# LongruiDong/nice-slam

Measured on AMD Instinct MI355X. Metric: ray-samples/sec (fwd+bwd) per mapping iter; frames/sec on Replica room0, higher is better.
Workload: dtype f32 (z, depth, var in f64); 1 GPU; Replica room0 mapping iteration, colour stage: 1000 pixels x 48 samples (5-frame window x 200), grids middle/fine/colour, Adam; global_batch=48000, seq_len=48, parallelism=rays sharded dp1, RCCL all-reduce of the frustum-row gradients

## Files before the change

include/nslam.h:

```cpp
#ifndef NSLAM_H
#define NSLAM_H

#include <stddef.h>
#include <stdint.h>

#ifdef __cplusplus
extern "C" {
#endif

#define NSLAM_C_DIM 32
#define NSLAM_HIDDEN 32
#define NSLAM_EMB 93

enum {
  NSLAM_OK = 0,
  NSLAM_EINVAL = -1,
  NSLAM_EUNSUPPORTED = -2,
  NSLAM_EWORKSPACE = -3,
  NSLAM_EHIP = -1000
};

enum { NSLAM_STAGE_COARSE = 0, NSLAM_STAGE_MIDDLE = 1, NSLAM_STAGE_FINE = 2, NSLAM_STAGE_COLOR = 3 };
enum { NSLAM_DEC_COARSE = 0, NSLAM_DEC_MIDDLE = 1, NSLAM_DEC_FINE = 2, NSLAM_DEC_COLOR = 3 };
enum { NSLAM_FWD_DEFAULT = 0, NSLAM_FWD_UNITS = 1, NSLAM_FWD_PC = 2, NSLAM_FWD_PARTS = 3 };
// ... 47 lines not shown
int nslam_query_fwd_ws(const nslam_query_cfg* cfg, const double* pts, int64_t n_pts, float* raw, void* ws,
                       size_t ws_bytes, void* stream);
size_t nslam_query_fwd_workspace_size(const nslam_query_cfg* cfg, int64_t n_pts);

int nslam_query_bwd(const nslam_query_cfg* cfg, const double* pts, int64_t n_pts, const float* g_raw,
                    double* g_pts, void* ws, size_t ws_bytes, void* stream);
size_t nslam_query_bwd_workspace_size(const nslam_query_cfg* cfg, int64_t n_pts);
int nslam_query_bwd_decoder(const nslam_query_cfg* cfg, int32_t dec, int32_t accumulate_pts, const double* pts,
                            int64_t n_pts, const float* g_raw, double* g_pts, void* ws, size_t ws_bytes,
                            void* stream);
size_t nslam_query_bwd_decoder_workspace_size(const nslam_query_cfg* cfg, int32_t dec, int64_t n_pts);
size_t nslam_query_saved_size(int64_t n_pts);
size_t nslam_query_tape_size(int64_t n_pts);
int nslam_query_bwd_decoders(const nslam_query_cfg* cfg, int32_t dec_mask, const double* pts, int64_t n_pts,
                             const float* g_raw, double* const* g_pts, void* stream);
int nslam_color_wgrad(const nslam_query_cfg* cfg, const double* pts, int64_t n_pts, const float* g_raw, void* ws,
                      size_t ws_bytes, void* stream);

int nslam_composite_fwd(const float* raw, const double* z_vals, int64_t n_rays, int32_t n_samples,
                        double* depth, double* var, float* color, void* stream);
int nslam_composite_bwd(const float* raw, const double* z_vals, int64_t n_rays, int32_t n_samples,
                        const double* g_depth, const double* g_var, const float* g_color, float* g_raw,
                        void* stream);

int nslam_grid_sample_fwd(const float* grid, const int32_t* dims, const float* coords, int64_t n,
                          float* out, void* stream);
int nslam_grid_sample_bwd(const float* grid, const int32_t* dims, const float* coords, int64_t n,
                          const float* grad_out, float* grad_grid, float* grad_coords, void* stream);

#define NSLAM_MAX_FRAMES 32
// ... 140 lines not shown
```

nice-slam_amd/_lib.py:

```python
from __future__ import annotations

import ctypes
import os

import torch

_HERE = os.path.dirname(os.path.abspath(__file__))
LIB_PATH = os.environ.get("NSLAM_LIB") or os.path.join(_HERE, "libnslam.so")

NSLAM_OK = 0
ABI_VERSION = 23
STAGES = {"coarse": 0, "middle": 1, "fine": 2, "color": 3}
DEC_COARSE, DEC_MIDDLE, DEC_FINE, DEC_COLOR = 0, 1, 2, 3

c_float_p = ctypes.POINTER(ctypes.c_float)


class NslamGrid(ctypes.Structure):
    _fields_ = [
        ("data", ctypes.c_void_p),
        ("grad", ctypes.c_void_p),
        ("dims", ctypes.c_int32 * 3),
        ("pad_", ctypes.c_int32),
        ("lo", ctypes.c_double * 3),
# ... 87 lines not shown

EXPORTS = (
    "nslam_pack_layout", "nslam_sample_rays", "nslam_query_fwd", "nslam_query_bwd", "nslam_query_bwd_workspace_size",
    "nslam_query_saved_size", "nslam_query_bwd_decoder", "nslam_query_bwd_decoder_workspace_size",
    "nslam_query_bwd_decoders",
    "nslam_composite_fwd", "nslam_composite_bwd", "nslam_grid_sample_fwd", "nslam_grid_sample_bwd",
    "nslam_workspace_size", "nslam_strerror", "nslam_abi_version", "nslam_gather_rays", "nslam_render_loss",
    "nslam_render_loss_workspace_size", "nslam_adam_step", "nslam_rows_pack", "nslam_rows_unpack",
    "nslam_query_fwd_ws", "nslam_query_fwd_workspace_size", "nslam_cam_grad", "nslam_cam_pose",
    "nslam_query_tape_size", "nslam_color_wgrad", "nslam_cam_grad_parts", "nslam_cam_grad_batch",
    "nslam_cam_pose_batch", "nslam_frustum_rows", "nslam_frustum_rows_workspace_size", "nslam_track_best",
    "nslam_loss_sum_best", "nslam_cam_vector_batch", "nslam_cam_grad_step",
    "nslam_point_masks", "nslam_point_masks_workspace_size", "nslam_mc_count", "nslam_mc_emit",
    "nslam_mc_workspace_size", "nslam_points_in_hull", "nslam_mesh_face_cull", "nslam_mesh_components",
    "nslam_mesh_select", "nslam_mesh_remap",
)

_lib = None


def lib():
    global _lib
    if _lib is None:
        if not os.path.exists(LIB_PATH):
            raise RuntimeError(f"{LIB_PATH} is missing: build it with __graft_entry__.build() "
                               "(make -C nice-slam_amd/csrc); there is no CPU fallback")
        L = ctypes.CDLL(LIB_PATH)
        missing = [n for n in EXPORTS if not hasattr(L, n)]
        if missing:
            raise RuntimeError(f"{LIB_PATH} does not export {', '.join(missing)}: rebuild it "
# ... 53 lines not shown
                                          vp, vp, vp, vp]
        f64 = ctypes.c_double
        L.nslam_point_masks.argtypes = [vp, i64, vp, i32, vp, i32, i32, f32, f32, f32, f32, i32, i32, i64, vp, vp, vp,
                                        vp, sz, vp]
        L.nslam_point_masks_workspace_size.argtypes = [i64, i32, i64]
        L.nslam_point_masks_workspace_size.restype = sz
        L.nslam_mc_count.argtypes = [vp, i32, i32, i32, f32, vp, sz, vp]
        L.nslam_mc_emit.argtypes = [vp, i32, i32, i32, f32, dp, dp, vp, vp, i64, i64, vp, vp, vp]
        L.nslam_mc_workspace_size.argtypes = [i32, i32, i32]
        L.nslam_mc_workspace_size.restype = sz
        L.nslam_points_in_hull.argtypes = [vp, i32, i64, vp, i32, vp, vp]
        L.nslam_mesh_face_cull.argtypes = [vp, i64, vp, i64, vp, vp]
        L.nslam_mesh_components.argtypes = [vp, i64, vp, i64, vp, vp, vp, vp]
        L.nslam_mesh_select.argtypes = [vp, i64, vp, vp, vp, f64, vp, vp, vp]
        L.nslam_mesh_remap.argtypes = [vp, i64, vp, vp, vp]
        if L.nslam_abi_version() != ABI_VERSION:
            raise RuntimeError(f"libnslam.so ABI {L.nslam_abi_version()} != {ABI_VERSION}: rebuild it")
        _lib = L
    return _lib


def check(rc: int, what: str):
    if rc != NSLAM_OK:
        msg = lib().nslam_strerror(rc).decode()
        raise RuntimeError(f"{what} failed: rc={rc} ({msg})")


def ptr(t):
    if t is None:
        return None
# ... 16 lines not shown
```

nice-slam_amd/csrc/nslam_query_impl.h:

```cpp
#pragma once
#include <type_traits>

#include "nslam_dev.h"

namespace nslamq {

struct QueryKArgs {
  nslam_query_cfg c;
  const double* pts;
  int64_t n;
  float* raw;
  const float* g_raw;
  double* g_pts;
};

struct Pt {
  double p[3];
  float x[3];
  bool valid;
  bool inside;
};

__device__ __forceinline__ Pt load_point(const QueryKArgs& a, int64_t idx) {
  Pt q;
// ... 267 lines not shown
__device__ __forceinline__ uint16_t* mask_slot(const QueryKArgs& a, int dec, int64_t tile) {
  const int64_t ntiles = (a.n + 31) / 32;
  return a.c.saved_masks + ((size_t)dec * ntiles + tile) * 5 * 64;
}
__device__ __forceinline__ void save_masks(const QueryKArgs& a, int dec, int64_t tile, const uint32_t m[5],
                                           int lane) {
  if (!a.c.saved_masks) return;
  uint16_t* s = mask_slot(a, dec, tile);
#pragma unroll
  for (int i = 0; i < 5; ++i) s[i * 64 + lane] = (uint16_t)m[i];
}
__device__ __forceinline__ void load_masks(const QueryKArgs& a, int dec, int64_t tile, uint32_t m[5], int lane) {
  const uint16_t* s = mask_slot(a, dec, tile);
#pragma unroll
  for (int i = 0; i < 5; ++i) m[i] = s[i * 64 + lane];
}

constexpr int kTapeFloats = 5 * 16 * 64;
__device__ __forceinline__ void tape_store(float* __restrict__ t, int i, const f32x16& v, int lane) {
  const int p = lane & 31, h = lane >> 5;
  __attribute__((address_space(1))) f32x4* q =
      reinterpret_cast<__attribute__((address_space(1))) f32x4*>(as_global_w(t) + i * 1024 + p * 32 + 4 * h);
#pragma unroll
  for (int k = 0; k < 4; ++k) q[2 * k] = f32x4{v[4 * k], v[4 * k + 1], v[4 * k + 2], v[4 * k + 3]};
}
struct Slab {
  __amdgpu_buffer_rsrc_t r;
};

__device__ __forceinline__ Slab make_slab(float* base, int floats) {
// ... 1321 lines not shown
static __global__ __launch_bounds__(256) void k_occ_combine(float* __restrict__ raw, const float* __restrict__ occ_mid,
                                                     int64_t n) {
  const int64_t p = (int64_t)blockIdx.x * 256 + threadIdx.x;
  if (p < n) raw[p * 4 + 3] = raw[p * 4 + 3] + occ_mid[p];
}

constexpr int kScratchFloats = 2 * TILE_FLOATS + 32 * 4 + 32 * 3 + 32 * 8 * 2 + 32;
constexpr int kWavesBwd = 4;
constexpr int kMaxSlabs = 4096;

constexpr bool lean_tr(int WG, bool PG, bool SAVED) { return SAVED && WG == 0 && !PG; }
constexpr int bwd_scratch_floats(int WG, bool PG, bool SAVED) {
  return WG ? kScratchFloats : lean_tr(WG, PG, SAVED) ? kWalkFloats : TILE_FLOATS + kWalkFloats;
}

template <int DEC, int WG, bool PG, bool FIRST, bool SAVED>
__device__ __forceinline__ void dec_bwd_tile(const QueryKArgs& a, int64_t tile, const Slab& A, const Scratch& S,
                                             int lane, double* __restrict__ gpts, int64_t gbase = 0) {
  asm volatile("" : "+v"(lane));
  PHASE(DEC, 0);
  const int h = lane >> 5, p = lane & 31;
  const int64_t idx = tile * 32 + p;
  const Pt q = load_point(a, idx);
  float g[4] = {0.f, 0.f, 0.f, 0.f};
  if (q.valid) {
    const f32x4 v = *reinterpret_cast<const f32x4*>(a.g_raw + idx * 4);
    g[0] = v[0];
    g[1] = v[1];
    g[2] = v[2];
    g[3] = q.inside ? v[3] : 0.f;
  }
  if (WG) {
    if (h == 0) {
#pragma unroll
      for (int j = 0; j < 4; ++j) S.gtab[p * 4 + j] = g[j];
#pragma unroll
      for (int j = 0; j < 3; ++j) S.xtab[p * 3 + j] = q.x[j];
// ... 8 lines not shown
  PHASE(DEC, 1);
  Corners cr;
  grid_corners(cr, gr, q);
  ScatterCorners scn{};
  if (WG == 0 && gr.grad) scn = resolve_corners(gr.slot, cr, q.valid, lane);
  PHASE(DEC, 2);
  f32x16 dc;
  float gx[3] = {0.f, 0.f, 0.f};
  static_assert(!(SAVED && WG), "weight gradients from saved masks run as k_color_wgrad");
  constexpr bool TR = lean_tr(WG, PG, SAVED);
  float* const tab = TR ? S.sA : S.sA + TILE_FLOATS;
  constexpr bool IMGDC = SAVED && WG == 0 && PG && DEC != NSLAM_DEC_COARSE;
  float* const img = IMGDC ? S.sA : nullptr;
  if (SAVED) {
    uint32_t m[5];
    load_masks(a, DEC, tile, m, lane);
    if (WG == 0 && gr.grad) stage_walk_table(tab, scn, cr.cell, lane);
    if (DEC == NSLAM_DEC_COARSE) {
      noxyz_backward_saved<TR>(pk, m, g[3], lane, dc);
    } else if (DEC == NSLAM_DEC_FINE) {
      xyz_backward_saved<2, 1, 3, PG, TR>(pk, m, q.x, g, lane, dc, gx, nullptr, img);
    } else if (DEC == NSLAM_DEC_COLOR) {
      xyz_backward_saved<1, 3, 0, PG, TR>(pk, m, q.x, g, lane, dc, gx, gh4, img);
    } else {
      xyz_backward_saved<1, 1, 3, PG, TR>(pk, m, q.x, g, lane, dc, gx, nullptr, img);
    }
  } else if (DEC == NSLAM_DEC_COARSE) {
    const f32x16 c = gather_tile(gr.data, cr, lane);
    noxyz_backward<WG>(pk, c, g[3], dg, A, S, lane, dc);
  } else if (DEC == NSLAM_DEC_FINE) {
    Corners cm;
// ... 80 lines not shown
      f32x4 t = s0[i];
      for (int v = 1; v < nv; ++v) t += s0[(size_t)v * q + i];
      s0[i] = t;
    }
    return;
  }
#pragma nounroll
  for (int64_t tile = w; tile < ntiles; tile += (int64_t)gridDim.x * kWavesBwd)
    dec_bwd_tile<DEC, WG, PG, FIRST, SAVED>(a, tile, A, S, lane, a.g_pts);
}

struct MultiDecArgs {
  int ndec;
  int dec[4];
  double* gp[4];
};
#ifndef NSLAM_MULTI_LB
#define NSLAM_MULTI_LB 4
#endif
#ifndef NSLAM_MULTI_PG_LB
#define NSLAM_MULTI_PG_LB 3
#endif
template <bool PG>
__global__ __launch_bounds__(64 * kWavesBwd, PG ? NSLAM_MULTI_PG_LB : NSLAM_MULTI_LB) void k_dec_bwd_multi(QueryKArgs a, MultiDecArgs m) {
  constexpr int kScr = bwd_scratch_floats(0, PG, true);
  __shared__ __attribute__((aligned(16))) float lds[kWavesBwd * kScr];
  const int lane = threadIdx.x & 63, wave = wave_id();
  Scratch S;
  S.sA = lds + wave * kScr;
  S.sX = S.gtab = S.xtab = S.cw = nullptr;
  S.crow = S.ccell = nullptr;
  const int part = (int)(blockIdx.x % (unsigned)m.ndec);
  const int dec = part == 0 ? m.dec[0] : part == 1 ? m.dec[1] : part == 2 ? m.dec[2] : m.dec[3];
  double* gp = part == 0 ? m.gp[0] : part == 1 ? m.gp[1] : part == 2 ? m.gp[2] : m.gp[3];
  const int64_t w = (int64_t)(blockIdx.x / (unsigned)m.ndec) * kWavesBwd + wave;
  const int64_t ntiles = (a.n + 31) / 32;
  if (w >= ntiles) return;
  TL(1, 0, part);
  const Slab A = make_slab(nullptr, 0);
  switch (dec) {
    case NSLAM_DEC_COARSE: dec_bwd_tile<NSLAM_DEC_COARSE, 0, PG, true, true>(a, w, A, S, lane, gp); break;
    case NSLAM_DEC_MIDDLE: dec_bwd_tile<NSLAM_DEC_MIDDLE, 0, PG, true, true>(a, w, A, S, lane, gp); break;
    case NSLAM_DEC_FINE: dec_bwd_tile<NSLAM_DEC_FINE, 0, PG, true, true>(a, w, A, S, lane, gp); break;
    default: dec_bwd_tile<NSLAM_DEC_COLOR, 0, PG, true, true>(a, w, A, S, lane, gp); break;
  }
  TL(1, 1, 0);
}

constexpr int kReduceWaves = 16;
static __global__ __launch_bounds__(64 * kReduceWaves) void k_slab_reduce(const float* __restrict__ slab, int64_t nslab,
                                                                   int acc_floats, int count,
                                                                   float* __restrict__ base) {
  __shared__ f32x4 part[kReduceWaves * 4][16];
  const int lane = threadIdx.x & 63, wave = wave_id();
  const int c = lane & 15, r = wave * 4 + (lane >> 4);
  const int j = (blockIdx.x * 16 + c) * 4;
  f32x4 s0 = {0.f, 0.f, 0.f, 0.f}, s1 = s0;
  if (j < count) {
    const float* p = slab + j;
// ... 188 lines not shown
```

nice-slam_amd/csrc/nslam_query_multi.hip:

```cpp
#include "nslam_query_impl.h"

using namespace nslamq;

extern "C" int nslam_query_bwd_decoders(const nslam_query_cfg* cfg, int32_t dec_mask, const double* pts,
                                        int64_t n_pts, const float* g_raw, double* const* g_pts, void* stream) {
  const int rc = check_cfg(cfg, true);
  if (rc) return rc;
  if (dec_mask <= 0 || dec_mask > 15) return NSLAM_EINVAL;
  if (n_pts < 0 || (n_pts > 0 && ((!pts && !cfg->rays_o) || !g_raw))) return NSLAM_EINVAL;
  if (cfg->rays_o && (n_pts >= (int64_t(1) << 31) || n_pts % cfg->n_samples)) return NSLAM_EINVAL;
  if (cfg->need_pts_grad && n_pts > 0 && !g_pts) return NSLAM_EINVAL;
  MultiDecArgs m{};
  for (int d = 0; d < 4; ++d) {
    if (!((dec_mask >> d) & 1)) continue;
    if (!stage_uses(cfg->stage, d)) return NSLAM_EINVAL;
    if (cfg->dgrad[d].base) return NSLAM_EUNSUPPORTED;
    if (cfg->need_pts_grad && n_pts > 0 && !g_pts[d]) return NSLAM_EINVAL;
    m.dec[m.ndec] = d;
    m.gp[m.ndec] = cfg->need_pts_grad ? g_pts[d] : nullptr;
    ++m.ndec;
  }
  if (n_pts > 0 && !cfg->saved_masks) return NSLAM_EUNSUPPORTED;
  if (n_pts == 0) return NSLAM_OK;
  const int64_t tiles = (n_pts + 31) / 32;
  const int64_t groups = (tiles + kWavesBwd - 1) / kWavesBwd;
  QueryKArgs a{*cfg, pts, n_pts, nullptr, g_raw, nullptr};
  hipStream_t s = reinterpret_cast<hipStream_t>(stream);
  const dim3 grid((unsigned)(groups * m.ndec)), block(64 * kWavesBwd);
  if (cfg->need_pts_grad)
    hipLaunchKernelGGL((k_dec_bwd_multi<true>), grid, block, 0, s, a, m);
  else
    hipLaunchKernelGGL((k_dec_bwd_multi<false>), grid, block, 0, s, a, m);
  return hip_status();
}

extern "C" int nslam_color_wgrad(const nslam_query_cfg* cfg, const double* pts, int64_t n_pts, const float* g_raw,
                                 void* ws, size_t ws_bytes, void* stream) {
  const int rc = check_cfg(cfg, true);
  if (rc) return rc;
  if (cfg->stage != NSLAM_STAGE_COLOR || n_pts < 0) return NSLAM_EINVAL;
  if (!cfg->dgrad[NSLAM_DEC_COLOR].base || cfg->dgrad[NSLAM_DEC_COLOR].count <= 0) return NSLAM_EUNSUPPORTED;
  if (n_pts > 0 && !cw_tape_path(cfg)) return NSLAM_EUNSUPPORTED;
  if (n_pts > 0 && ((!pts && !cfg->rays_o) || !g_raw)) return NSLAM_EINVAL;
  if (cfg->rays_o && (n_pts >= (int64_t(1) << 31) || n_pts % cfg->n_samples)) return NSLAM_EINVAL;
  if (n_pts == 0) return NSLAM_OK;
  if (!ws || ws_bytes < dec_ws_bytes(cfg, NSLAM_DEC_COLOR, n_pts)) return NSLAM_EWORKSPACE;
  QueryKArgs a{*cfg, pts, n_pts, nullptr, g_raw, nullptr};
  return launch_color_wgrad(a, reinterpret_cast<float*>(ws), reinterpret_cast<hipStream_t>(stream));
}
```

nice-slam_amd/engine.py:

```python
from __future__ import annotations

import ctypes
import math
import os
import weakref

import numpy as np
import torch

from . import _lib, ops
from ._lib import check, lib, ptr, stream_ptr
from .common import get_camera_from_tensor

_GRID_OF = {"coarse": "grid_coarse", "middle": "grid_middle", "fine": "grid_fine", "color": "grid_color"}


def _env_choice(name, default, allowed):
    v = os.environ.get(name, default)
    if v not in allowed:
        raise ValueError(f"{name}={v!r}: expected one of {sorted(allowed)}")
    return v


class FlatDecoder:
# ... 39 lines not shown
                 rows=None):
        self.nice, self.c, self.bound = nice, c, bound
        self.n_strat, self.n_surf, self.lindisp, self.w_color = n_strat, n_surf, lindisp, w_color
        self.device = torch.device(device)
        names = [n for n in ("coarse", "middle", "fine", "color") if hasattr(nice, n + "_decoder")]
        self.decs = {n: FlatDecoder(nice.decoder(n)) for n in names}
        self.dec_bounds = {n: ops._bound_list(nice.decoder(n).bound) for n in names}
        self.oob = ops._bound_list(bound)
        self._saved = None
        self._tape = None
        self.occ_add = None
        self._draws = None
        self._pre = None
        self._parity = 0
        self._pre_stream = None
        self._side = []
        self.concurrent = True
        self.wgrad_first = _env_choice("NSLAM_WGRAD_FIRST", "1", ("0", "1")) == "1"
        self.merge = True
        self._lean_ev = None
        self.prefetch_at = _env_choice("NSLAM_PREFETCH_AT", "start", ("start", "after_fwd"))
        self.prefetch_stream = _env_choice("NSLAM_PREFETCH_STREAM", "lean", ("lean", "own"))
        self.adam_merge = _env_choice("NSLAM_ADAM_MERGE", "1", ("0", "1")) == "1"
        self.adam_on = _env_choice("NSLAM_ADAM_ON", "side", ("side", "main"))
        self._wg_ev = None
        for k, v in c.items():
            if not v.is_contiguous(memory_format=torch.channels_last_3d):
                raise ValueError(f"{k} must be channels-last (ops.channels_last)")
        self.grid_grads = grid_grads
        self.layout_gen = 0
        self.pad_rows = 1
        self.set_rows(rows)

    def set_rows(self, rows, pad_rows=None):
        c = self.c
        pad = max(1, int(self.pad_rows if pad_rows is None else pad_rows))
        self.layout_gen += 1
        rup = lambda n: -(-n // pad) * pad
        drup = lambda n: -(-n // (32 * pad)) * 32 * pad
        self.rows = dict(rows) if rows else {}
# ... 36 lines not shown
        keys = tuple(sorted(masks))
        if getattr(self, "_cap_keys", None) != keys:
            self._cap = {}
            rows = {}
            for k in keys:
                n = self.c[k].numel() // 32
                full = torch.empty(n + 1, dtype=torch.int32, device=self.device)
                full[:n] = torch.arange(n, dtype=torch.int32, device=self.device)
                self._cap[k] = (full, torch.full((1,), n, dtype=torch.int64, device=self.device),
                                torch.arange(n, dtype=torch.int32, device=self.device))
                rows[k] = full[:n]
            self.set_rows(rows, pad_rows=1)
            self._cap_keys = keys
            self.gall.zero_()
            self._clean = True
        for k in keys:
            full, n_live, ar = self._cap[k]
            n = ar.numel()
            m = masks[k]
            if m is None:
                full[:n].copy_(ar)
                self.slot[k].copy_(ar)
                n_live.fill_(n)
                continue
            m = m.permute(2, 1, 0).reshape(-1)
            idx = torch.cumsum(m, 0, dtype=torch.int32) - 1
            self.slot[k].copy_(torch.where(m, idx, torch.full_like(idx, -1)))
            full.scatter_(0, torch.where(m, idx, torch.full_like(idx, n)).long(), ar)
            n_live.copy_(idx[-1:].to(torch.int64) + 1)
        return {k: self._cap[k][1] for k in keys}
# ... 7 lines not shown
        meta = ops.QueryMeta(stage, decs, {n: self.decs[n].packer for n in decs},
                             {n: self.dec_bounds[n] for n in decs}, self.oob, None)
        pairs = [(None, None, None)] * 4
        for n in decs:
            key = _GRID_OF[n]
            gg = key in grid_grads
            pairs[ops._DEC_ID[n]] = (self.c[key], self.ggrad[key] if gg else None, self.slot.get(key) if gg else None)
        packed = {n: self.decs[n].packed for n in decs}
        dg = {n: self.decs[n].grad for n in decs if n in dec_grads}
        cfg = ops._fill_cfg(meta, pairs, packed, dg, False)
        cfg.rays_o, cfg.rays_d, cfg.z_vals, cfg.n_samples = ptr(ro), ptr(rd), ptr(z), z.shape[1]
        cfg.saved_masks = ptr(self._saved)
        cfg.act_tape = ptr(self._tape)
        return cfg

    def query_fwd(self, stage, ro, rd, z, defer_occ=False, tape=False):
        n = z.numel()
        raw = torch.empty(n, 4, dtype=torch.float32, device=z.device)
        self._saved = torch.empty(lib().nslam_query_saved_size(n), dtype=torch.uint8, device=z.device)
        self._tape = None
        if tape and stage == "color":
            self._tape = torch.empty(lib().nslam_query_tape_size(n) // 4, dtype=torch.float32, device=z.device)
        cfg = self._cfg(stage, ro, rd, z, (), ())
        self.occ_add = ops.query_fwd_launch(cfg, None, n, raw, defer_occ=defer_occ)
        return raw

    def query_bwd(self, stage, ro, rd, z, g_raw, grid_grads, dec_grads, concurrent=None, pts_grad=False,
                  on_branch=None, pts_parts=False, ordered_branches=False, on_pts=None):
        n = z.numel()
        self._clean = False
        concurrent = self.concurrent if concurrent is None else concurrent
        cfg = self._cfg(stage, ro, rd, z, grid_grads, dec_grads)
        cfg.need_pts_grad = int(bool(pts_grad))
        decs = list(ops._DEC_FOR_STAGE[stage])
        wgt = [d for d in decs if d in dec_grads]
        masks = self._saved is not None
        tape_color = "color" in wgt and masks and self._tape is not None
        lean = [d for d in decs if self.merge and masks and (d not in wgt or (d == "color" and tape_color))]
        others = [d for d in decs if d not in lean]
        gp = {d: torch.empty(n, 3, dtype=torch.float64, device=z.device) for d in decs} if pts_grad else None
        units = []
        if "color" in lean and "color" in wgt and n > 0:
            units.append(("wgrad", ["color"]))
        if lean:
            units.append(("lean", lean))
        units += [("one", [d]) for d in others]
        if not self.wgrad_first:
            units.sort(key=lambda u: u[0] == "wgrad")
# ... 1 lines not shown
        merged_names = None
        merge_adam = (self.adam_merge and has_wgrad and on_branch is not None and not ordered_branches
                      and self.wgrad_first and concurrent and len(units) == 2 and units[1][0] == "lean")
        wgrad_st = None
        main = torch.cuda.current_stream(z.device)
        par = concurrent and len(units) > 1
        streams = [main]
        if par:
            while len(self._side) < len(units) - 1:
                self._side.append(torch.cuda.Stream(z.device))
            streams += self._side[:len(units) - 1]
        used = streams[1:]
        with ops._span("query_bwd"):
            for st in used:
                st.wait_stream(main)
                for t in (ro, rd, z, g_raw, self._saved, self._tape):
                    if t is not None:
                        t.record_stream(st)
            for i, (kind, names) in enumerate(units):
                st = streams[i] if par else main
                with torch.cuda.stream(st):
                    if kind == "wgrad":
                        wsb = lib().nslam_query_bwd_decoder_workspace_size(ctypes.byref(cfg), _lib.DEC_COLOR, n)
                        ws = torch.empty(wsb, dtype=torch.uint8, device=z.device)
                        with ops._span("query_bwd.color_wgrad"):
                            rc = lib().nslam_color_wgrad(ctypes.byref(cfg), None, n, ptr(g_raw), ptr(ws), wsb,
                                                         st.cuda_stream)
                        check(rc, "nslam_color_wgrad")
                        wgrad_st = st
                        if merge_adam:
                            if self._wg_ev is None:
                                self._wg_ev = torch.cuda.Event()
                            self._wg_ev.record(st)
                    elif kind == "lean":
                        lc = _lib.NslamQueryCfg.from_buffer_copy(cfg)
                        gps = (ctypes.c_void_p * 4)()
                        mask = 0
                        for name in names:
                            d = ops._DEC_ID[name]
                            mask |= 1 << d
                            lc.dgrad[d] = _lib.NslamDecGrad()
                            if pts_grad:
                                gps[d] = ptr(gp[name])
                        with ops._span("query_bwd." + "+".join(names)):
                            rc = lib().nslam_query_bwd_decoders(ctypes.byref(lc), mask, None, n, ptr(g_raw), gps,
                                                                st.cuda_stream)
                        check(rc, "nslam_query_bwd_decoders")
                        if on_pts is not None and pts_grad and set(names) == set(decs):
                            for name in names:
                                gp[name].record_stream(st)
                            on_pts([gp[d] for d in decs])
                            on_pts = None
                        if has_wgrad and self._lean_ev is None:
                            self._lean_ev = torch.cuda.Event()
                        if has_wgrad and not ordered_branches:
                            self._lean_ev.record(st)
                        if on_branch is not None and merge_adam and self.adam_on == "main":
                            merged_names = names
                        elif on_branch is not None and merge_adam:
                            st.wait_event(self._wg_ev)
                            on_branch(names, part="all")
# ... 53 lines not shown
    def adam_grads(self, stage, trainable_decoders):
        keys, dnames = self.grads_for(stage, trainable_decoders)
        g = {self.c[k]: self.ggrad[k] for k in keys}
        g.update({self.decs[n].param: self.decs[n].grad for n in dnames})
        return g

    def iteration(self, stage, frames, pix, n_per, hw, intrinsics, optimizer, trainable_decoders=("color",),
                  gt_max=None, allreduce=None, use_gt_in_sampler=True, exchange=None, n_kept=None, seed=0,
                  world=1, rank=0, prefetch=False, post_bwd=None):
        H, W = hw
        fx, fy, cx, cy = intrinsics
        keys, dnames = self.grads_for(stage, trainable_decoders)
        if exchange is not None and hasattr(exchange, "validate"):
            exchange.validate(self, keys, dnames)
        draw = self.draws(seed, world, rank) if pix is None else None

        def rays(out=None):
            ro, rd, gd, gc, keep = ops.gather_rays(frames, pix, n_per, H, W, (0, H, 0, W), fx, fy, cx, cy,
                                                   self.bound, draw=draw, n_kept=n_kept,
                                                   out=None if out is None else out[:5])
            gsamp = gd if (use_gt_in_sampler and stage != "coarse") else None
            if gsamp is None:
                gm = None
            elif draw is not None and draw.gt_max is not None:
                gm = draw.gt_max
            else:
                gm = gt_max(gd) if gt_max is not None else None
            z = ops.sample_z(ro, rd, gsamp, self.bound, self.n_strat, self.n_surf, self.lindisp, gt_max=gm,
                             out=None if out is None else out[5])
            return [ro, rd, gd, gc, keep, z]

        prefetch = prefetch and pix is None
        side = None
        if prefetch:
            ftens = [t for f in frames for t in f]
            pkey = (stage, n_per, hw, use_gt_in_sampler, seed, world, rank)
            valid = (self._pre is not None and self._pre[0] == pkey and len(self._pre[1]) == len(ftens)
                     and all(r() is t and v == t._version for (r, v), t in zip(self._pre[1], ftens)))
            if not valid:
                first = rays()
                self._pre = (pkey, [(weakref.ref(t), t._version) for t in ftens],
                             [first, [torch.empty_like(t) for t in first]])
                self._parity = 0
            cur, nxt = self._pre[2][self._parity], self._pre[2][1 - self._parity]
            self._parity ^= 1
            main = torch.cuda.current_stream(self.device)
            if self._pre_stream is None:
                if self.prefetch_stream == "lean" and self.wgrad_first and self.concurrent:
                    if not self._side:
                        self._side.append(torch.cuda.Stream(self.device))
                    self._pre_stream = self._side[0]
                else:
                    self._pre_stream = torch.cuda.Stream(self.device)
            side = self._pre_stream

            def launch_prefetch():
                side.wait_stream(main)
                with torch.cuda.stream(side):
                    rays(out=nxt)

            if self.prefetch_at == "start":
                launch_prefetch()
            ro, rd, gd, gc, keep, z = cur
        else:
            ro, rd, gd, gc, keep, z = rays()
        mirror = hasattr(optimizer, "set_mirror")
        raw = self.query_fwd(stage, ro, rd, z, defer_occ=True, tape="color" in dnames)
        if side is not None and self.prefetch_at != "start":
            launch_prefetch()
        _, _, _, ray_loss, g_raw = ops.render_loss(raw, z, gd, gc, keep, mode="mapper", use_color=stage == "color",
                                                   w_color=self.w_color, occ_add=self.occ_add)
        if not self._clean:
            self.gall.zero_()
        clean = all(k in self.rows for k in keys)
        if mirror:
            for n in dnames:
                d = self.decs[n]
                if d.param not in optimizer.mirrors:
                    optimizer.set_mirror(d.param, d.mirror_idx, d.packed)
        grads = self.adam_grads(stage, trainable_decoders)
# ... 3 lines not shown
            def on_branch(names, part=None):
                exchange.branch(names, part, keys, dnames)
        elif exchange is None and allreduce is None and mirror:
            def on_branch(names, part=None):
                sub = {}
                for name in names:
                    if _GRID_OF[name] in keys and part != "decoders":
                        sub[self.c[_GRID_OF[name]]] = grads[self.c[_GRID_OF[name]]]
                    if name in dnames and part != "grids":
                        sub[self.decs[name].param] = grads[self.decs[name].param]
                if sub:
                    optimizer.step(grads=sub, zero_grad=clean)

        on_pts = (lambda parts: post_bwd(parts, ro, rd, z)) if post_bwd is not None else None
        self.query_bwd(stage, ro, rd, z, g_raw, keys, dnames, on_branch=on_branch, ordered_branches=sharded,
                       pts_grad=post_bwd is not None, pts_parts=True, on_pts=on_pts)
        if sharded:
            pass
        elif exchange is not None:
            exchange(keys, dnames)
        elif allreduce is not None:
            allreduce([self.gbuf] + [self.decs[n].grad for n in dnames])
        if side is not None:
            main.wait_stream(side)
        if on_branch is None:
            optimizer.step(grads=grads, zero_grad=clean)
        self._clean = clean and (not sharded or exchange.leaves_clean)
        if not mirror:
            for n in dnames:
                self.decs[n].repack()
        return ray_loss, keep
# ... 101 lines not shown
```

nice-slam_amd/mapper.py:

```python
from __future__ import annotations

import numpy as np
import torch

from . import common as _common
from . import ops
from .common import get_camera_from_tensor, get_samples, get_tensor_from_camera, random_select

_SELECT_UV = _common.select_uv
_STAGE_GROUPS = ("decoders", "coarse", "middle", "fine", "color")


def _remap_bilinear(img, u, v):
    H, W = img.shape
    X = torch.round(u.clamp(-1e8, 1e8) * 32).to(torch.int64)
    Y = torch.round(v.clamp(-1e8, 1e8) * 32).to(torch.int64)
    x0, y0 = torch.div(X, 32, rounding_mode="floor"), torch.div(Y, 32, rounding_mode="floor")
    fx = (X - x0 * 32).to(torch.float32) / 32
    fy = (Y - y0 * 32).to(torch.float32) / 32

    def tap(x, y):
        ok = (x >= 0) & (x < W) & (y >= 0) & (y < H)
        return torch.where(ok, img[y.clamp(0, H - 1), x.clamp(0, W - 1)], torch.zeros((), device=img.device))

# ... 257 lines not shown
            n = max(F, self.mapping_window_size)
            self._slots = (torch.zeros(n, H, W, dtype=torch.float32, device=dev),
                           torch.zeros(n, H, W, 3, dtype=torch.float32, device=dev),
                           torch.eye(4, dtype=torch.float32, device=dev).repeat(n, 1, 1))
            self._graphs.clear()
        return self._slots

    def _bind_frustum(self, eng, c2w, depth):
        keys = self._grid_keys()
        if (not self.frustum_feature_selection or self.coarse_mapper
                or "get_mask_from_c2w" in self.__dict__):
            eng.bind_masks(self._call_masks(c2w, depth))
            return
        if getattr(eng, "_cap_keys", None) != tuple(sorted(keys)):
            eng.bind_masks({k: None for k in keys})
        done = {}
        for k in keys:
            shp = tuple(self.c[k].shape[2:])
            rows, n_live = eng.live_rows(k)
            slot = eng.slot[k]
            if shp in done:
                s0, r0, n0 = done[shp]
                slot.copy_(s0)
                rows.copy_(r0)
                n_live.copy_(n0)
            else:
                frustum_rows_device(c2w, shp, depth, self.bound, self.H, self.W, self.fx, self.fy, self.cx, self.cy,
                                    slot, rows, n_live)
                done[shp] = (slot, rows, n_live)

# ... 377 lines not shown
```

Before: 234.7 million ray-samples/s.

## Compact live sample points per decoder and skip dead tiles in backward

Adds a flag/scan/emit kernel chain that builds, per decoder, a compacted index list of sample points whose grid corners touch frustum-live rows. The mask-only mapping backward then iterates only over those live points, so tiles whose points cannot contribute grid gradients are never launched. Live lists are cached with the prefetched ray batch and invalidated by a rows/layout generation counter. The cost is three extra small kernels per batch and indexed, non-coalesced point and mask loads in the backward.

Result: faster. 244.1 million ray-samples/s (median of 6 runs) (+4.0%).

```diff
diff --git a/include/nslam.h b/include/nslam.h
--- a/include/nslam.h
+++ b/include/nslam.h
@@ -85,6 +85,12 @@
 size_t nslam_query_tape_size(int64_t n_pts);
 int nslam_query_bwd_decoders(const nslam_query_cfg* cfg, int32_t dec_mask, const double* pts, int64_t n_pts,
                              const float* g_raw, double* const* g_pts, void* stream);
+int nslam_live_points(const nslam_query_cfg* cfg, int32_t dec_mask, const double* pts, int64_t n_pts,
+                      int32_t* const* live_idx, int64_t* const* n_live, void* ws, size_t ws_bytes, void* stream);
+size_t nslam_live_points_workspace_size(int64_t n_pts);
+int nslam_query_bwd_decoders_live(const nslam_query_cfg* cfg, int32_t dec_mask, const double* pts, int64_t n_pts,
+                                  const float* g_raw, const int32_t* const* live_idx, const int64_t* const* n_live,
+                                  void* stream);
 int nslam_color_wgrad(const nslam_query_cfg* cfg, const double* pts, int64_t n_pts, const float* g_raw, void* ws,
                       size_t ws_bytes, void* stream);
 
diff --git a/nice-slam_amd/_lib.py b/nice-slam_amd/_lib.py
--- a/nice-slam_amd/_lib.py
+++ b/nice-slam_amd/_lib.py
@@ -125,6 +125,7 @@
     "nslam_point_masks", "nslam_point_masks_workspace_size", "nslam_mc_count", "nslam_mc_emit",
     "nslam_mc_workspace_size", "nslam_points_in_hull", "nslam_mesh_face_cull", "nslam_mesh_components",
     "nslam_mesh_select", "nslam_mesh_remap",
+    "nslam_live_points", "nslam_live_points_workspace_size", "nslam_query_bwd_decoders_live",
 )
 
 _lib = None
@@ -208,6 +209,12 @@
         L.nslam_mesh_components.argtypes = [vp, i64, vp, i64, vp, vp, vp, vp]
         L.nslam_mesh_select.argtypes = [vp, i64, vp, vp, vp, f64, vp, vp, vp]
         L.nslam_mesh_remap.argtypes = [vp, i64, vp, vp, vp]
+        L.nslam_live_points.argtypes = [ctypes.POINTER(NslamQueryCfg), i32, vp, i64, ctypes.POINTER(vp),
+                                        ctypes.POINTER(vp), vp, sz, vp]
+        L.nslam_live_points_workspace_size.argtypes = [i64]
+        L.nslam_live_points_workspace_size.restype = sz
+        L.nslam_query_bwd_decoders_live.argtypes = [ctypes.POINTER(NslamQueryCfg), i32, vp, i64, vp,
+                                                    ctypes.POINTER(vp), ctypes.POINTER(vp), vp]
         if L.nslam_abi_version() != ABI_VERSION:
             raise RuntimeError(f"libnslam.so ABI {L.nslam_abi_version()} != {ABI_VERSION}: rebuild it")
         _lib = L
diff --git a/nice-slam_amd/csrc/nslam_query_impl.h b/nice-slam_amd/csrc/nslam_query_impl.h
--- a/nice-slam_amd/csrc/nslam_query_impl.h
+++ b/nice-slam_amd/csrc/nslam_query_impl.h
@@ -305,6 +305,11 @@
   const uint16_t* s = mask_slot(a, dec, tile);
 #pragma unroll
   for (int i = 0; i < 5; ++i) m[i] = s[i * 64 + lane];
+}
+__device__ __forceinline__ void load_masks_at(const QueryKArgs& a, int dec, int64_t idx, int h, uint32_t m[5]) {
+  const uint16_t* s = mask_slot(a, dec, idx >> 5) + ((int)(idx & 31) | (h << 5));
+#pragma unroll
+  for (int i = 0; i < 5; ++i) m[i] = s[i * 64];
 }
 
 constexpr int kTapeFloats = 5 * 16 * 64;
@@ -1656,13 +1661,19 @@
   return WG ? kScratchFloats : lean_tr(WG, PG, SAVED) ? kWalkFloats : TILE_FLOATS + kWalkFloats;
 }
 
-template <int DEC, int WG, bool PG, bool FIRST, bool SAVED>
+template <int DEC, int WG, bool PG, bool FIRST, bool SAVED, bool LIVE = false>
 __device__ __forceinline__ void dec_bwd_tile(const QueryKArgs& a, int64_t tile, const Slab& A, const Scratch& S,
-                                             int lane, double* __restrict__ gpts, int64_t gbase = 0) {
+                                             int lane, double* __restrict__ gpts, int64_t gbase = 0,
+                                             const int32_t* __restrict__ live = nullptr, int64_t nlive = 0) {
+  static_assert(!LIVE || (SAVED && WG == 0 && !PG), "live-point tiles: the mask-only mapping backward");
   asm volatile("" : "+v"(lane));
   PHASE(DEC, 0);
   const int h = lane >> 5, p = lane & 31;
-  const int64_t idx = tile * 32 + p;
+  int64_t idx = tile * 32 + p;
+  if (LIVE) {
+    const uint32_t v = idx < nlive ? (uint32_t)live[idx] : 0xffffffffu;
+    idx = (int64_t)v < a.n ? (int64_t)v : a.n;
+  }
   const Pt q = load_point(a, idx);
   float g[4] = {0.f, 0.f, 0.f, 0.f};
   if (q.valid) {
@@ -1701,7 +1712,10 @@
   float* const img = IMGDC ? S.sA : nullptr;
   if (SAVED) {
     uint32_t m[5];
-    load_masks(a, DEC, tile, m, lane);
+    if (LIVE)
+      load_masks_at(a, DEC, q.valid ? idx : 0, h, m);
+    else
+      load_masks(a, DEC, tile, m, lane);
     if (WG == 0 && gr.grad) stage_walk_table(tab, scn, cr.cell, lane);
     if (DEC == NSLAM_DEC_COARSE) {
       noxyz_backward_saved<TR>(pk, m, g[3], lane, dc);
@@ -1812,6 +1826,8 @@
   int ndec;
   int dec[4];
   double* gp[4];
+  const int32_t* live[4];
+  const int64_t* nlive[4];
 };
 #ifndef NSLAM_MULTI_LB
 #define NSLAM_MULTI_LB 4
@@ -1819,8 +1835,9 @@
 #ifndef NSLAM_MULTI_PG_LB
 #define NSLAM_MULTI_PG_LB 3
 #endif
-template <bool PG>
+template <bool PG, bool LIVE = false>
 __global__ __launch_bounds__(64 * kWavesBwd, PG ? NSLAM_MULTI_PG_LB : NSLAM_MULTI_LB) void k_dec_bwd_multi(QueryKArgs a, MultiDecArgs m) {
+  static_assert(!(PG && LIVE), "d/dpts is needed for every point");
   constexpr int kScr = bwd_scratch_floats(0, PG, true);
   __shared__ __attribute__((aligned(16))) float lds[kWavesBwd * kScr];
   const int lane = threadIdx.x & 63, wave = wave_id();
@@ -1832,15 +1849,29 @@
   const int dec = part == 0 ? m.dec[0] : part == 1 ? m.dec[1] : part == 2 ? m.dec[2] : m.dec[3];
   double* gp = part == 0 ? m.gp[0] : part == 1 ? m.gp[1] : part == 2 ? m.gp[2] : m.gp[3];
   const int64_t w = (int64_t)(blockIdx.x / (unsigned)m.ndec) * kWavesBwd + wave;
-  const int64_t ntiles = (a.n + 31) / 32;
+  const int32_t* live = nullptr;
+  int64_t nlive = a.n;
+  if (LIVE) {
+    live = part == 0 ? m.live[0] : part == 1 ? m.live[1] : part == 2 ? m.live[2] : m.live[3];
+    const int64_t* np = part == 0 ? m.nlive[0] : part == 1 ? m.nlive[1] : part == 2 ? m.nlive[2] : m.nlive[3];
+    nlive = *np;
+    if (nlive > a.n) nlive = a.n;
+  }
+  const int64_t ntiles = (nlive + 31) / 32;
   if (w >= ntiles) return;
   TL(1, 0, part);
   const Slab A = make_slab(nullptr, 0);
   switch (dec) {
-    case NSLAM_DEC_COARSE: dec_bwd_tile<NSLAM_DEC_COARSE, 0, PG, true, true>(a, w, A, S, lane, gp); break;
-    case NSLAM_DEC_MIDDLE: dec_bwd_tile<NSLAM_DEC_MIDDLE, 0, PG, true, true>(a, w, A, S, lane, gp); break;
-    case NSLAM_DEC_FINE: dec_bwd_tile<NSLAM_DEC_FINE, 0, PG, true, true>(a, w, A, S, lane, gp); break;
-    default: dec_bwd_tile<NSLAM_DEC_COLOR, 0, PG, true, true>(a, w, A, S, lane, gp); break;
+    case NSLAM_DEC_COARSE:
+      dec_bwd_tile<NSLAM_DEC_COARSE, 0, PG, true, true, LIVE>(a, w, A, S, lane, gp, 0, live, nlive);
+      break;
+    case NSLAM_DEC_MIDDLE:
+      dec_bwd_tile<NSLAM_DEC_MIDDLE, 0, PG, true, true, LIVE>(a, w, A, S, lane, gp, 0, live, nlive);
+      break;
+    case NSLAM_DEC_FINE:
+      dec_bwd_tile<NSLAM_DEC_FINE, 0, PG, true, true, LIVE>(a, w, A, S, lane, gp, 0, live, nlive);
+      break;
+    default: dec_bwd_tile<NSLAM_DEC_COLOR, 0, PG, true, true, LIVE>(a, w, A, S, lane, gp, 0, live, nlive); break;
   }
   TL(1, 1, 0);
 }
diff --git a/nice-slam_amd/csrc/nslam_query_multi.hip b/nice-slam_amd/csrc/nslam_query_multi.hip
--- a/nice-slam_amd/csrc/nslam_query_multi.hip
+++ b/nice-slam_amd/csrc/nslam_query_multi.hip
@@ -34,6 +34,165 @@
   return hip_status();
 }
 
+namespace {
+constexpr int kLiveBlock = 256;
+
+struct LiveArgs {
+  int ndec;
+  int dec[4];
+  int32_t* idx[4];
+  int64_t* n[4];
+};
+struct LiveWs {
+  uint64_t* ballot;
+  uint32_t* count;
+  int64_t nwaves, nblocks;
+};
+
+__global__ __launch_bounds__(kLiveBlock) void k_live_flags(QueryKArgs a, LiveArgs m, LiveWs w) {
+  __shared__ uint32_t wc[kLiveBlock / 64];
+  const int part = (int)blockIdx.y;
+  const int dec = part == 0 ? m.dec[0] : part == 1 ? m.dec[1] : part == 2 ? m.dec[2] : m.dec[3];
+  const int64_t idx = (int64_t)blockIdx.x * kLiveBlock + threadIdx.x;
+  const Pt q = load_point(a, idx);
+  const nslam_grid& gr = a.c.grid[dec];
+  bool live = q.valid;
+  if (gr.slot) {
+    Corners cr;
+    grid_corners(cr, gr, q);
+    bool any = false;
+#pragma unroll
+    for (int k = 0; k < 8; ++k)
+      any = any || (((cr.ok >> k) & 1u) && gr.slot[cr.row[k]] >= 0);
+    live = live && any;
+  }
+  const uint64_t b = __ballot(live);
+  const int wave = wave_id();
+  if ((threadIdx.x & 63) == 0) {
+    w.ballot[(size_t)part * w.nwaves + (size_t)blockIdx.x * (kLiveBlock / 64) + wave] = b;
+    wc[wave] = (uint32_t)__popcll(b);
+  }
+  __syncthreads();
+  if (threadIdx.x == 0) w.count[(size_t)part * w.nblocks + blockIdx.x] = (wc[0] + wc[1]) + (wc[2] + wc[3]);
+}
+
+__global__ __launch_bounds__(256) void k_live_scan(LiveArgs m, LiveWs w) {
+  __shared__ uint32_t sh[256];
+  const int part = (int)blockIdx.x;
+  int64_t* nout = part == 0 ? m.n[0] : part == 1 ? m.n[1] : part == 2 ? m.n[2] : m.n[3];
+  uint32_t* c = w.count + (size_t)part * w.nblocks;
+  const int t = (int)threadIdx.x;
+  uint32_t carry = 0;
+  for (int64_t base = 0; base < w.nblocks; base += 256) {
+    const int64_t i = base + t;
+    const uint32_t v = i < w.nblocks ? c[i] : 0u;
+    sh[t] = v;
+    __syncthreads();
+    for (int d = 1; d < 256; d <<= 1) {
+      const uint32_t add = t >= d ? sh[t - d] : 0u;
+      __syncthreads();
+      sh[t] += add;
+      __syncthreads();
+    }
+    if (i < w.nblocks) c[i] = carry + sh[t] - v;
+    carry += sh[255];
+    __syncthreads();
+  }
+  if (t == 0) *nout = (int64_t)carry;
+}
+
+__global__ __launch_bounds__(kLiveBlock) void k_live_emit(int64_t n, LiveArgs m, LiveWs w) {
+  const int part = (int)blockIdx.y;
+  int32_t* out = part == 0 ? m.idx[0] : part == 1 ? m.idx[1] : part == 2 ? m.idx[2] : m.idx[3];
+  const int64_t idx = (int64_t)blockIdx.x * kLiveBlock + threadIdx.x;
+  const int wave = wave_id(), lane = threadIdx.x & 63;
+  const uint64_t* bw = w.ballot + (size_t)part * w.nwaves + (size_t)blockIdx.x * (kLiveBlock / 64);
+  uint32_t pos = w.count[(size_t)part * w.nblocks + blockIdx.x];
+  for (int v = 0; v < wave; ++v) pos += (uint32_t)__popcll(bw[v]);
+  const uint64_t b = bw[wave];
+  if (!((b >> lane) & 1)) return;
+  pos += (uint32_t)__popcll(b & ((uint64_t(1) << lane) - 1));
+  if (idx < n && (int64_t)pos < n) out[pos] = (int32_t)idx;
+}
+
+inline int64_t live_nblocks(int64_t n) { return (n + kLiveBlock - 1) / kLiveBlock; }
+inline size_t live_ws_bytes(int64_t n) {
+  const int64_t nb = live_nblocks(n);
+  return n > 0 ? (size_t)4 * ((size_t)nb * (kLiveBlock / 64) * 8 + (size_t)nb * 4) : 0;
+}
+}
+
+extern "C" size_t nslam_live_points_workspace_size(int64_t n_pts) { return live_ws_bytes(n_pts); }
+
+extern "C" int nslam_live_points(const nslam_query_cfg* cfg, int32_t dec_mask, const double* pts, int64_t n_pts,
+                                 int32_t* const* live_idx, int64_t* const* n_live, void* ws, size_t ws_bytes,
+                                 void* stream) {
+  const int rc = check_cfg(cfg, true);
+  if (rc) return rc;
+  if (dec_mask <= 0 || dec_mask > 15 || !live_idx || !n_live) return NSLAM_EINVAL;
+  if (n_pts < 0 || n_pts >= (int64_t(1) << 31) || (n_pts > 0 && !pts && !cfg->rays_o)) return NSLAM_EINVAL;
+  if (cfg->rays_o && n_pts % cfg->n_samples) return NSLAM_EINVAL;
+  LiveArgs m{};
+  for (int d = 0; d < 4; ++d) {
+    if (!((dec_mask >> d) & 1)) continue;
+    if (!stage_uses(cfg->stage, d)) return NSLAM_EINVAL;
+    if (!n_live[d] || (n_pts > 0 && !live_idx[d])) return NSLAM_EINVAL;
+    m.dec[m.ndec] = d;
+    m.idx[m.ndec] = live_idx[d];
+    m.n[m.ndec] = n_live[d];
+    ++m.ndec;
+  }
+  hipStream_t s = reinterpret_cast<hipStream_t>(stream);
+  if (n_pts == 0) {
+    for (int i = 0; i < m.ndec; ++i)
+      if (hipMemsetAsync(m.n[i], 0, sizeof(int64_t), s) != hipSuccess) return hip_status();
+    return NSLAM_OK;
+  }
+  if (!ws || ws_bytes < live_ws_bytes(n_pts) || (((uintptr_t)ws) & 7) != 0) return NSLAM_EWORKSPACE;
+  LiveWs w;
+  w.nblocks = live_nblocks(n_pts);
+  w.nwaves = w.nblocks * (kLiveBlock / 64);
+  w.ballot = reinterpret_cast<uint64_t*>(ws);
+  w.count = reinterpret_cast<uint32_t*>(w.ballot + (size_t)4 * w.nwaves);
+  QueryKArgs a{*cfg, pts, n_pts, nullptr, nullptr, nullptr};
+  const dim3 grid((unsigned)w.nblocks, (unsigned)m.ndec);
+  hipLaunchKernelGGL(k_live_flags, grid, dim3(kLiveBlock), 0, s, a, m, w);
+  hipLaunchKernelGGL(k_live_scan, dim3((unsigned)m.ndec), dim3(256), 0, s, m, w);
+  hipLaunchKernelGGL(k_live_emit, grid, dim3(kLiveBlock), 0, s, n_pts, m, w);
+  return hip_status();
+}
+
+extern "C" int nslam_query_bwd_decoders_live(const nslam_query_cfg* cfg, int32_t dec_mask, const double* pts,
+                                             int64_t n_pts, const float* g_raw, const int32_t* const* live_idx,
+                                             const int64_t* const* n_live, void* stream) {
+  const int rc = check_cfg(cfg, true);
+  if (rc) return rc;
+  if (dec_mask <= 0 || dec_mask > 15 || !live_idx || !n_live) return NSLAM_EINVAL;
+  if (n_pts < 0 || (n_pts > 0 && ((!pts && !cfg->rays_o) || !g_raw))) return NSLAM_EINVAL;
+  if (n_pts >= (int64_t(1) << 31) || (cfg->rays_o && n_pts % cfg->n_samples)) return NSLAM_EINVAL;
+  if (cfg->need_pts_grad) return NSLAM_EUNSUPPORTED;
+  MultiDecArgs m{};
+  for (int d = 0; d < 4; ++d) {
+    if (!((dec_mask >> d) & 1)) continue;
+    if (!stage_uses(cfg->stage, d)) return NSLAM_EINVAL;
+    if (cfg->dgrad[d].base) return NSLAM_EUNSUPPORTED;
+    if (!n_live[d] || (n_pts > 0 && !live_idx[d])) return NSLAM_EINVAL;
+    m.dec[m.ndec] = d;
+    m.live[m.ndec] = live_idx[d];
+    m.nlive[m.ndec] = n_live[d];
+    ++m.ndec;
+  }
+  if (n_pts > 0 && !cfg->saved_masks) return NSLAM_EUNSUPPORTED;
+  if (n_pts == 0) return NSLAM_OK;
+  const int64_t tiles = (n_pts + 31) / 32;
+  const int64_t groups = (tiles + kWavesBwd - 1) / kWavesBwd;
+  QueryKArgs a{*cfg, pts, n_pts, nullptr, g_raw, nullptr};
+  hipStream_t s = reinterpret_cast<hipStream_t>(stream);
+  const dim3 grid((unsigned)(groups * m.ndec)), block(64 * kWavesBwd);
+  hipLaunchKernelGGL((k_dec_bwd_multi<false, true>), grid, block, 0, s, a, m);
+  return hip_status();
+}
+
 extern "C" int nslam_color_wgrad(const nslam_query_cfg* cfg, const double* pts, int64_t n_pts, const float* g_raw,
                                  void* ws, size_t ws_bytes, void* stream) {
   const int rc = check_cfg(cfg, true);
diff --git a/nice-slam_amd/engine.py b/nice-slam_amd/engine.py
--- a/nice-slam_amd/engine.py
+++ b/nice-slam_amd/engine.py
@@ -77,6 +77,7 @@
         self._pre = None
         self._parity = 0
         self._pre_stream = None
+        self._live_gen = [None, None]
         self._side = []
         self.concurrent = True
         self.wgrad_first = _env_choice("NSLAM_WGRAD_FIRST", "1", ("0", "1")) == "1"
@@ -87,6 +88,8 @@
         self.adam_merge = _env_choice("NSLAM_ADAM_MERGE", "1", ("0", "1")) == "1"
         self.adam_on = _env_choice("NSLAM_ADAM_ON", "side", ("side", "main"))
         self._wg_ev = None
+        self.live_points = _env_choice("NSLAM_LIVE_POINTS", "1", ("0", "1")) == "1"
+        self.rows_gen = 0
         for k, v in c.items():
             if not v.is_contiguous(memory_format=torch.channels_last_3d):
                 raise ValueError(f"{k} must be channels-last (ops.channels_last)")
@@ -153,6 +156,7 @@
             self._cap_keys = keys
             self.gall.zero_()
             self._clean = True
+        self.rows_gen += 1
         for k in keys:
             full, n_live, ar = self._cap[k]
             n = ar.numel()
@@ -190,6 +194,34 @@
         cfg.act_tape = ptr(self._tape)
         return cfg
 
+    def live_lists(self, stage, ro, rd, z, out=None):
+        decs = ops._DEC_FOR_STAGE[stage]
+        n = z.numel()
+        if out is None:
+            out = (torch.empty(len(decs), n, dtype=torch.int32, device=z.device),
+                   torch.zeros(4, dtype=torch.int64, device=z.device))
+        idx, nl = out
+        keys = tuple(_GRID_OF[d] for d in decs) if self.grid_grads else ()
+        saved, tape = self._saved, self._tape
+        self._saved = self._tape = None
+        try:
+            cfg = self._cfg(stage, ro, rd, z, keys, ())
+        finally:
+            self._saved, self._tape = saved, tape
+        ips, nps = (ctypes.c_void_p * 4)(), (ctypes.c_void_p * 4)()
+        mask = 0
+        for i, name in enumerate(decs):
+            d = ops._DEC_ID[name]
+            mask |= 1 << d
+            ips[d] = idx[i].data_ptr()
+            nps[d] = nl[d:d + 1].data_ptr()
+        wsb = lib().nslam_live_points_workspace_size(n)
+        ws = torch.empty(max(wsb, 8), dtype=torch.uint8, device=z.device)
+        with ops._span("live_points"):
+            rc = lib().nslam_live_points(ctypes.byref(cfg), mask, None, n, ips, nps, ptr(ws), wsb, stream_ptr(z.device))
+        check(rc, "nslam_live_points")
+        return idx, nl
+
     def query_fwd(self, stage, ro, rd, z, defer_occ=False, tape=False):
         n = z.numel()
         raw = torch.empty(n, 4, dtype=torch.float32, device=z.device)
@@ -202,12 +234,14 @@
         return raw
 
     def query_bwd(self, stage, ro, rd, z, g_raw, grid_grads, dec_grads, concurrent=None, pts_grad=False,
-                  on_branch=None, pts_parts=False, ordered_branches=False, on_pts=None):
+                  on_branch=None, pts_parts=False, ordered_branches=False, on_pts=None, live=None):
         n = z.numel()
         self._clean = False
         concurrent = self.concurrent if concurrent is None else concurrent
         cfg = self._cfg(stage, ro, rd, z, grid_grads, dec_grads)
         cfg.need_pts_grad = int(bool(pts_grad))
+        if pts_grad:
+            live = None
         decs = list(ops._DEC_FOR_STAGE[stage])
         wgt = [d for d in decs if d in dec_grads]
         masks = self._saved is not None
@@ -239,7 +273,7 @@
         with ops._span("query_bwd"):
             for st in used:
                 st.wait_stream(main)
-                for t in (ro, rd, z, g_raw, self._saved, self._tape):
+                for t in (ro, rd, z, g_raw, self._saved, self._tape) + (tuple(live) if live else ()):
                     if t is not None:
                         t.record_stream(st)
             for i, (kind, names) in enumerate(units):
@@ -268,8 +302,17 @@
                             if pts_grad:
                                 gps[d] = ptr(gp[name])
                         with ops._span("query_bwd." + "+".join(names)):
-                            rc = lib().nslam_query_bwd_decoders(ctypes.byref(lc), mask, None, n, ptr(g_raw), gps,
-                                                                st.cuda_stream)
+                            if live is not None:
+                                ips, nps = (ctypes.c_void_p * 4)(), (ctypes.c_void_p * 4)()
+                                for name in names:
+                                    d = ops._DEC_ID[name]
+                                    ips[d] = live[0][decs.index(name)].data_ptr()
+                                    nps[d] = live[1][d:d + 1].data_ptr()
+                                rc = lib().nslam_query_bwd_decoders_live(ctypes.byref(lc), mask, None, n, ptr(g_raw),
+                                                                         ips, nps, st.cuda_stream)
+                            else:
+                                rc = lib().nslam_query_bwd_decoders(ctypes.byref(lc), mask, None, n, ptr(g_raw),
+                                                                    gps, st.cuda_stream)
                         check(rc, "nslam_query_bwd_decoders")
                         if on_pts is not None and pts_grad and set(names) == set(decs):
                             for name in names:
@@ -353,6 +396,8 @@
         if exchange is not None and hasattr(exchange, "validate"):
             exchange.validate(self, keys, dnames)
         draw = self.draws(seed, world, rank) if pix is None else None
+        use_live = (self.live_points and post_bwd is None and self.grid_grads and self.merge
+                    and any(k in self.slot for k in keys))
 
         def rays(out=None):
             ro, rd, gd, gc, keep = ops.gather_rays(frames, pix, n_per, H, W, (0, H, 0, W), fx, fy, cx, cy,
@@ -367,13 +412,15 @@
                 gm = gt_max(gd) if gt_max is not None else None
             z = ops.sample_z(ro, rd, gsamp, self.bound, self.n_strat, self.n_surf, self.lindisp, gt_max=gm,
                              out=None if out is None else out[5])
-            return [ro, rd, gd, gc, keep, z]
+            lv = list(self.live_lists(stage, ro, rd, z, out=None if out is None else out[6:8])) if use_live else []
+            return [ro, rd, gd, gc, keep, z] + lv
 
         prefetch = prefetch and pix is None
         side = None
         if prefetch:
             ftens = [t for f in frames for t in f]
-            pkey = (stage, n_per, hw, use_gt_in_sampler, seed, world, rank)
+            pkey = (stage, n_per, hw, use_gt_in_sampler, seed, world, rank, use_live)
+            gen = (self.layout_gen, self.rows_gen)
             valid = (self._pre is not None and self._pre[0] == pkey and len(self._pre[1]) == len(ftens)
                      and all(r() is t and v == t._version for (r, v), t in zip(self._pre[1], ftens)))
             if not valid:
@@ -381,8 +428,13 @@
                 self._pre = (pkey, [(weakref.ref(t), t._version) for t in ftens],
                              [first, [torch.empty_like(t) for t in first]])
                 self._parity = 0
-            cur, nxt = self._pre[2][self._parity], self._pre[2][1 - self._parity]
+                self._live_gen = [gen, None]
+            par = self._parity
+            cur, nxt = self._pre[2][par], self._pre[2][1 - par]
             self._parity ^= 1
+            if use_live and self._live_gen[par] != gen:
+                self.live_lists(stage, cur[0], cur[1], cur[5], out=cur[6:8])
+                self._live_gen[par] = gen
             main = torch.cuda.current_stream(self.device)
             if self._pre_stream is None:
                 if self.prefetch_stream == "lean" and self.wgrad_first and self.concurrent:
@@ -397,12 +449,15 @@
                 side.wait_stream(main)
                 with torch.cuda.stream(side):
                     rays(out=nxt)
+                self._live_gen[1 - par] = gen
 
             if self.prefetch_at == "start":
                 launch_prefetch()
-            ro, rd, gd, gc, keep, z = cur
+            batch = cur
         else:
-            ro, rd, gd, gc, keep, z = rays()
+            batch = rays()
+        ro, rd, gd, gc, keep, z = batch[:6]
+        live = tuple(batch[6:8]) if use_live else None
         mirror = hasattr(optimizer, "set_mirror")
         raw = self.query_fwd(stage, ro, rd, z, defer_occ=True, tape="color" in dnames)
         if side is not None and self.prefetch_at != "start":
@@ -436,7 +491,7 @@
 
         on_pts = (lambda parts: post_bwd(parts, ro, rd, z)) if post_bwd is not None else None
         self.query_bwd(stage, ro, rd, z, g_raw, keys, dnames, on_branch=on_branch, ordered_branches=sharded,
-                       pts_grad=post_bwd is not None, pts_parts=True, on_pts=on_pts)
+                       pts_grad=post_bwd is not None, pts_parts=True, on_pts=on_pts, live=live)
         if sharded:
             pass
         elif exchange is not None:
diff --git a/nice-slam_amd/mapper.py b/nice-slam_amd/mapper.py
--- a/nice-slam_amd/mapper.py
+++ b/nice-slam_amd/mapper.py
@@ -295,6 +295,7 @@
             return
         if getattr(eng, "_cap_keys", None) != tuple(sorted(keys)):
             eng.bind_masks({k: None for k in keys})
+        eng.rows_gen += 1
         done = {}
         for k in keys:
             shp = tuple(self.c[k].shape[2:])
```
